# TUMFTM/RadarGNN

Hardware: AMD Instinct MI355X
Metric: radar frames/sec (graph-build + GNN fwd) (higher is better)
Workload: dtype f32 (dense layers: fp32 operands split into 2 f16 terms after an exact power-of-two pre-scale, 3 f16 MFMA products per fp32 product, fp32 accumulate -- more accurate than fp32 MFMA against float64, tests/test_gpu_f16x2.py; RGNN_NO_F16X2=1 selects 3 bf16 terms / 6 products, RGNN_LINEAR_FP32=1 v_mfma_; 1 GPU; C2: per GPU 64 RadarScenes-shaped frames x 3000 pts, radius graph r=1.0, node feats [rcs,velocity_vector,time_index,degree], edge feats [relative_position], 4-layer MPNNConv [224,224,128,64] + emb MLPs + both heads, train-mode BatchNorm, max aggr; frames_per_gpu=64, points_per_gpu=192000, edges_per_gpu=799078, ranks_in_process_group=1

## Files before the change

### radargnn_amd/csrc/mpnn_tiles.hip

```cpp
#include "common.h"
#include <stdlib.h>
#include <type_traits>

namespace {

constexpr int MT_THREADS = 256;
constexpr int MT_WAVES = MT_THREADS / 64;
constexpr int MT_QUEUE_INTS = 8 * 16;

typedef float mt_f32x16 __attribute__((ext_vector_type(16)));
typedef __bf16 mt_bf16x8 __attribute__((ext_vector_type(8)));
typedef unsigned int mt_u32x4 __attribute__((ext_vector_type(4)));

__global__ __launch_bounds__(256) void k_tiles_zero_empty(const int32_t* __restrict__ rowptr, const int32_t* __restrict__ order,
                                                         int64_t n, int d, float* __restrict__ out, int64_t ldo) {
  const int lane = threadIdx.x & 63;
  const int64_t p = (int64_t)blockIdx.x * MT_WAVES + (threadIdx.x >> 6);
  if (p >= n || rowptr[p + 1] != rowptr[p]) return;
  const int64_t node = order ? order[p] : p;
  for (int c = lane; c < d; c += 64) out[node * ldo + c] = 0.f;
}

__device__ __forceinline__ void mt_split3(float x, unsigned& t1, unsigned& t2, unsigned& t3) {
  t1 = __float_as_uint(x) & 0xffff0000u;
  const float r = x - __uint_as_float(t1);
  t2 = __float_as_uint(r) & 0xffff0000u;
  const float r2 = r - __uint_as_float(t2);
  t3 = __float_as_uint(r2) & 0xffff0000u;
}
__device__ __forceinline__ unsigned mt_pack(unsigned lo, unsigned hi) { return (lo >> 16) | hi; }
__device__ __forceinline__ void mt_split_row(const float (&x)[8], mt_u32x4& p1, mt_u32x4& p2, mt_u32x4& p3) {
  unsigned t1[8], t2[8], t3[8];
#pragma unroll
  for (int k = 0; k < 8; k++) mt_split3(x[k], t1[k], t2[k], t3[k]);
  p1 = mt_u32x4{mt_pack(t1[0], t1[1]), mt_pack(t1[2], t1[3]), mt_pack(t1[4], t1[5]), mt_pack(t1[6], t1[7])};
  p2 = mt_u32x4{mt_pack(t2[0], t2[1]), mt_pack(t2[2], t2[3]), mt_pack(t2[4], t2[5]), mt_pack(t2[6], t2[7])};
  p3 = mt_u32x4{mt_pack(t3[0], t3[1]), mt_pack(t3[2], t3[3]), mt_pack(t3[4], t3[5]), mt_pack(t3[6], t3[7])};
}

}

namespace {

constexpr int WN_SLOTS = 512;
constexpr int WN_THREADS = 256;
typedef int wn_i32x4 __attribute__((ext_vector_type(4)));

struct WinParams {
  const float* p_bias;
  const float* Q; int ldq4; int q_bytes;
  const mt_u32x4* wplanes;
  const float* ea; int de; int ea_vec;
  int n_win;
  const int32_t* n_win_dev;
  const int32_t* plan; int plan_bytes;
  int off_misc;
  int off_eid;
  int off_lrow;
  int off_urow;
  int off_tgt;
  int32_t* queue;
  int d; int n_ct;
  float* out; int ldo4; int o_bytes;
  float* out_absmax;
  int abl;
};

__device__ __forceinline__ void wn_dma16(wn_i32x4 rsrc, int voff, int soff, unsigned lds_base) {
  asm volatile(
      "s_mov_b32 m0, %3\n\t"
      "s_nop 0\n\t"
      "buffer_load_dwordx4 %0, %1, %2 offen lds"
      :
      : "v"(voff), "s"(rsrc), "s"(soff), "s"(lds_base)
      : "memory");
}

__global__ __launch_bounds__(256) void k_win_wplanes(const float* __restrict__ We, int ldwe, int de, int d, int n_ct, const float* __restrict__ p_bias,
                                                     mt_u32x4* __restrict__ planes) {
  const int c = blockIdx.x * blockDim.x + threadIdx.x;
  if (c >= n_ct * 32) return;
  float w[8];
#pragma unroll
  for (int k = 0; k < 8; k++) w[k] = (c < d && k < de) ? We[(int64_t)c * ldwe + k] : 0.f;
  mt_u32x4 p1, p2, p3;
  mt_split_row(w, p1, p2, p3);
  mt_u32x4* t = planes + (c >> 5) * 128 + (c & 31);
  t[0] = p1; t[32] = p2; t[64] = p3;
  t[96] = mt_u32x4{__float_as_uint((p_bias != nullptr && c < d) ? p_bias[c] : 0.f), 0u, 0u, 0u};
}

constexpr int WN_PAD = 4;
constexpr int WN_GPT = 16 / WN_PAD;
constexpr int WN_GPS = 64 / WN_PAD;
constexpr int WN_TMAX = 512 / WN_PAD;
static_assert(WN_PAD == 2 || WN_PAD == 4, "segments are padded to 2 or 4 slots");
constexpr int WN_NOEND = (int)0x80000000u;
constexpr int WN_UMAX = 176;
constexpr int WN_ROWBUF = WN_UMAX * 128;

__device__ __forceinline__ void wn_wait_leaving(int n) {
  switch (n) {
#define WN_W(N) case N: asm volatile("s_waitcnt vmcnt(" #N ")" ::: "memory"); break;
    WN_W(1) WN_W(2) WN_W(3) WN_W(4) WN_W(5) WN_W(6) WN_W(7) WN_W(8) WN_W(9) WN_W(10) WN_W(11) WN_W(12) WN_W(13) WN_W(14) WN_W(15) WN_W(16)
    WN_W(17) WN_W(18) WN_W(19) WN_W(20) WN_W(21) WN_W(22) WN_W(23) WN_W(24) WN_W(25) WN_W(26) WN_W(27) WN_W(28) WN_W(29) WN_W(30) WN_W(31) WN_W(32)
#undef WN_W
    default: asm volatile("s_waitcnt vmcnt(0)" ::: "memory"); break;
  }
}

constexpr bool WN_WARM = false;
constexpr int WN_BBUF = 32 * 64;

constexpr int WN_DESC = 2 * WN_UMAX * 4 + 2048 + 512 + 8 * WN_GPS * 4 + 64;
static_assert((2 * WN_UMAX * 128 + 2 * 32 * 64 + WN_DESC + 16 + 511) / 512 * 512 * 3 <= 160 * 1024, "k_mpnn_win: LDS of three work-groups per CU");
constexpr int WN_LDS = 2 * WN_ROWBUF + 2 * WN_BBUF + WN_DESC + 16;

template <bool AMAX>
__global__ __launch_bounds__(WN_THREADS) __attribute__((amdgpu_waves_per_eu(3, 3))) void k_mpnn_win(const WinParams p) {
  extern __shared__ __attribute__((aligned(16))) char smem[];
  char* bstage = smem + 2 * WN_ROWBUF;
  int* urowtab = (int*)(bstage + 2 * WN_BBUF);
  int* eidtab = urowtab + 2 * WN_UMAX;
  const uint8_t* lrowtab = (const uint8_t*)(eidtab + 512);
  int* tgttab = eidtab + 512 + 128;
  int* misctab = tgttab + 8 * WN_GPS;
  int* bcast = misctab + 16;
  const unsigned rows_lds = (unsigned)(uintptr_t)(__attribute__((address_space(3))) char*)smem;
  const unsigned b_lds = rows_lds + 2 * WN_ROWBUF;
  const unsigned desc_lds = b_lds + 2 * WN_BBUF;
  const int tid = threadIdx.x, lane = tid & 63, wave = __builtin_amdgcn_readfirstlane(tid >> 6), half = lane >> 5, col = lane & 31, col4 = col * 4;
  const int xcd = blockIdx.x & 7;
  const int n_win = min(p.n_win, __builtin_amdgcn_readfirstlane(p.n_win_dev[0]));
  const int i_lo = (int)((int64_t)n_win * xcd / 8), i_hi = (int)((int64_t)n_win * (xcd + 1) / 8);
  int32_t* ticket = p.queue + xcd * 16;
  wn_i32x4 rq, rw, rp;
  {
    const uint64_t a = (uint64_t)p.Q;
    rq.x = __builtin_amdgcn_readfirstlane((int)(uint32_t)a);
    rq.y = __builtin_amdgcn_readfirstlane((int)(uint32_t)((a >> 32) & 0xffff));
    rq.z = __builtin_amdgcn_readfirstlane(p.q_bytes);
    rq.w = 0x00020000;
    const uint64_t b = (uint64_t)p.wplanes;
    rw.x = __builtin_amdgcn_readfirstlane((int)(uint32_t)b);
    rw.y = __builtin_amdgcn_readfirstlane((int)(uint32_t)((b >> 32) & 0xffff));
    rw.z = __builtin_amdgcn_readfirstlane(p.n_ct * WN_BBUF);
    rw.w = 0x00020000;
    const uint64_t c = (uint64_t)p.plan;
    rp.x = __builtin_amdgcn_readfirstlane((int)(uint32_t)c);
    rp.y = __builtin_amdgcn_readfirstlane((int)(uint32_t)((c >> 32) & 0xffff));
    rp.z = __builtin_amdgcn_readfirstlane(p.plan_bytes);
    rp.w = 0x00020000;
  }
  const int rA = lane & 31, hA = (rA >> 2) & 1, iA = ((rA >> 3) << 2) | (rA & 3);
  const int my_stream = 2 * wave + half;
  float amax = 0.f;

  auto desc_dma = [&](const int w, const int up) {
    if (wave == 0) {
      if (lane < WN_UMAX / 4) wn_dma16(rp, lane * 16, __builtin_amdgcn_readfirstlane(p.off_urow + w * (WN_UMAX * 4)),
                                       (unsigned)__builtin_amdgcn_readfirstlane((int)(desc_lds + up * (WN_UMAX * 4))));
    } else if (wave == 1) {
      wn_dma16(rp, lane * 16, __builtin_amdgcn_readfirstlane(p.off_eid + w * 2048), desc_lds + 8 * WN_UMAX);
      wn_dma16(rp, lane * 16, __builtin_amdgcn_readfirstlane(p.off_eid + w * 2048 + 1024), desc_lds + 8 * WN_UMAX + 1024);
    } else if (wave == 2) {
      if (lane < 32) wn_dma16(rp, lane * 16, __builtin_amdgcn_readfirstlane(p.off_lrow + w * 512), desc_lds + 8 * WN_UMAX + 2048);
    } else {
      if (lane < 2 * WN_GPS) wn_dma16(rp, lane * 16, __builtin_amdgcn_readfirstlane(p.off_tgt + w * (32 * WN_GPS)), desc_lds + 8 * WN_UMAX + 2560);
      if (lane < 4) wn_dma16(rp, lane * 16, __builtin_amdgcn_readfirstlane(p.off_misc + w * 64), desc_lds + 8 * WN_UMAX + 2560 + 32 * WN_GPS);
    }
  };
  auto stage = [&](const int ct, const int st, const int up, const int nU8) {
    const unsigned base = rows_lds + st * WN_ROWBUF;
    const int* ut = urowtab + up * WN_UMAX;
    for (int k = wave; k < nU8; k += 4)
      wn_dma16(rq, (int)__umul24((unsigned)ut[8 * k + (lane >> 3)], (unsigned)p.ldq4) + (lane & 7) * 16, __builtin_amdgcn_readfirstlane(ct * 128),
               (unsigned)__builtin_amdgcn_readfirstlane((int)(base + k * 1024)));
    if (wave == 1) {
      const unsigned bb = b_lds + st * WN_BBUF;
      wn_dma16(rw, lane * 16, __builtin_amdgcn_readfirstlane(ct * WN_BBUF), (unsigned)__builtin_amdgcn_readfirstlane((int)bb));
      wn_dma16(rw, lane * 16 + 1024, __builtin_amdgcn_readfirstlane(ct * WN_BBUF), (unsigned)__builtin_amdgcn_readfirstlane((int)(bb + 1024)));
    }
  };

  if (tid == 0) { bcast[0] = i_lo + atomicAdd(ticket, 1); bcast[1] = i_lo + atomicAdd(ticket, 1); }
  __syncthreads();
  int win = bcast[0];
  int up = 0;
  int gp = 0;
  bool staged = false;
  if (win < i_hi) desc_dma(win, 0);
  asm volatile("s_waitcnt vmcnt(0)" ::: "memory");
  __syncthreads();
  for (;;) {
    if (win >= i_hi) {
      if (tid == 0) {
        const int wgs = (int)(gridDim.x >> 3);
        if (atomicAdd(ticket + 1, 1) == wgs - 1) { ticket[0] = 0; ticket[1] = 0; }
      }
      break;
    }
    const int nxt = bcast[1];
    const int nU = misctab[0];
    const int nU8 = (nU + 7) >> 3;
    int nt = 0;
    unsigned anyend = 0;
    mt_u32x4 a1[4], a2[4], a3[4];
    int aoff[4][16];
    int tv = WN_NOEND;
    if (nU != 0) {
      const uint8_t* m8 = (const uint8_t*)(misctab + 1);
      nt = max((int)m8[2 * wave], (int)m8[2 * wave + 1]);
      const uint8_t* e4 = m8 + 8 + my_stream * 4;
      const unsigned endbits = (unsigned)e4[0] | ((unsigned)e4[1] << WN_GPT) | ((unsigned)e4[2] << (2 * WN_GPT)) | ((unsigned)e4[3] << (3 * WN_GPT));
      anyend = (unsigned)__builtin_amdgcn_readlane((int)endbits, 0) | (unsigned)__builtin_amdgcn_readlane((int)endbits, 32);
      const int gj = lane & (WN_GPS - 1);
      tv = ((endbits >> gj) & 1u) ? tgttab[my_stream * WN_GPS + gj] * p.ldo4 : WN_NOEND;
#pragma unroll
      for (int t = 0; t < 4; t++) {
        const int e = eidtab[(2 * wave + hA) * 64 + t * 16 + iA];
        float z[8];
        if (p.ea_vec) {
          const float4 mine = *(const float4*)(p.ea + (int64_t)e * 8 + half * 4);
          const float4 other = make_float4(__shfl_xor(mine.x, 32, 64), __shfl_xor(mine.y, 32, 64), __shfl_xor(mine.z, 32, 64), __shfl_xor(mine.w, 32, 64));
          const float4 lo = half ? other : mine, hi = half ? mine : other;
          z[0] = lo.x; z[1] = lo.y; z[2] = lo.z; z[3] = lo.w; z[4] = hi.x; z[5] = hi.y; z[6] = hi.z; z[7] = hi.w;
        } else {
#pragma unroll
          for (int k = 0; k < 8; k++) z[k] = (k < p.de) ? p.ea[(int64_t)e * p.de + k] : 0.f;
        }
        mt_u32x4 t3;
        mt_split_row(z, a1[t], a2[t], t3);
        a3[t] = half ? a1[t] : t3;
      }
      const mt_u32x4* lt = (const mt_u32x4*)(lrowtab + my_stream * 64);
#pragma unroll
      for (int t = 0; t < 4; t++) {
        const mt_u32x4 w4 = lt[t];
#pragma unroll
        for (int i = 0; i < 16; i++) {
          const unsigned w = w4[i >> 2];
          const unsigned r = (i & 3) == 3 ? (w >> 24) : ((w >> (8 * (i & 3))) & 0xffu);
          aoff[t][i] = (int)(rows_lds + (r << 7)) + col4;
          asm volatile("" : "+v"(aoff[t][i]));
        }
      }
    }
    __syncthreads();
    if (tid == 0) bcast[1] = i_lo + atomicAdd(ticket, 1);
    if (nU == 0) {
      if (nxt < i_hi) desc_dma(nxt, up ^ 1);
      asm volatile("s_waitcnt vmcnt(0)" ::: "memory");
      __syncthreads();
      win = nxt; up ^= 1; staged = false;
      continue;
    }
    const int nst = __builtin_popcount(anyend & ((nt >= 4) ? (WN_GPT == 8 ? 0xffffffffu : 0xffffu) : ((1u << (WN_GPT * nt)) - 1u)));
    if (!staged) stage(0, gp, up, nU8);
    bool staged_next = false;

    auto tile_pass = [&](const int ct, auto stage_c) {
      constexpr int ST = decltype(stage_c)::value;
      if (ct == 0 || (p.abl & 1)) asm volatile("s_waitcnt vmcnt(0)" ::: "memory");
      else wn_wait_leaving(nst);
      __syncthreads();
      if (ct == 0 && nxt < i_hi) desc_dma(nxt, up ^ 1);
      if (ct + 1 < p.n_ct) {
        if (!(p.abl & 1)) stage(ct + 1, ST ^ 1, up, nU8);
      } else if (ct > 0 && nxt < i_hi && !(p.abl & 1)) {
        const int nUn = misctab[0];
        if (nUn != 0) { stage(0, ST ^ 1, up ^ 1, (nUn + 7) >> 3); staged_next = true; }
      }
      const mt_u32x4* bl = (const mt_u32x4*)(bstage + ST * WN_BBUF);
      const mt_u32x4 bxc = bl[(half ? 32 : 0) + col], byc = bl[(half ? 64 : 0) + col];
      const float biasc = __uint_as_float(bl[96 + col].x);
      const int voffc = (ct * 32 + col < p.d && !(p.abl & 4)) ? col4 : 0x7ffffff0;
      const __amdgpu_buffer_rsrc_t ro_l = __builtin_amdgcn_make_buffer_rsrc((void*)((char*)p.out + ct * 128), (short)0, p.o_bytes - ct * 128, 0x00020000);
      float rn = -INFINITY;
      asm volatile("" : "+v"(tv), "+s"(anyend));
#pragma unroll
      for (int t = 0; t < 4; t++) {
        if (t < nt && !(p.abl & 2)) {
          mt_f32x16 c;
#pragma unroll
          for (int i = 0; i < 16; i++) c[i] = *(const __attribute__((address_space(3))) float*)(uintptr_t)(unsigned)(aoff[t][i] + ST * WN_ROWBUF);
          c = __builtin_amdgcn_mfma_f32_32x32x16_bf16(__builtin_bit_cast(mt_bf16x8, a3[t]), __builtin_bit_cast(mt_bf16x8, byc), c, 0, 0, 0);
          c = __builtin_amdgcn_mfma_f32_32x32x16_bf16(__builtin_bit_cast(mt_bf16x8, a2[t]), __builtin_bit_cast(mt_bf16x8, bxc), c, 0, 0, 0);
          c = __builtin_amdgcn_mfma_f32_32x32x16_bf16(__builtin_bit_cast(mt_bf16x8, a1[t]), __builtin_bit_cast(mt_bf16x8, bxc), c, 0, 0, 0);
#pragma unroll
          for (int g = 0; g < WN_GPT; g++) {
            rn = __builtin_fmaxf(__builtin_fmaxf(rn, c[WN_PAD * g]), c[WN_PAD * g + 1]);
            if (WN_PAD == 4) rn = __builtin_fmaxf(__builtin_fmaxf(rn, c[WN_PAD * g + 2]), c[WN_PAD * g + 3]);
            if ((anyend >> (WN_GPT * t + g)) & 1u) {
              const float v = rn + biasc;
              const int toA = __builtin_amdgcn_readlane(tv, WN_GPT * t + g), toB = __builtin_amdgcn_readlane(tv, 32 + WN_GPT * t + g);
              const int tog = half ? toB : toA;
              asm volatile("buffer_store_dword %0, %1, %2, 0 offen nt" : : "v"(v), "v"((unsigned)tog + (unsigned)voffc), "s"(ro_l) : "memory");
              if (AMAX) amax = fmaxf(amax, fabsf(v));
              rn = (tog >= 0) ? -INFINITY : rn;
            }
          }
        }
      }
    };
    float amax_full = 0.f;
    for (int ct = 0; ct < p.n_ct; ct++) {
      const bool partial = AMAX && (ct + 1) * 32 > p.d;
      if (partial) { amax_full = amax; amax = 0.f; }
      if ((gp + ct) & 1) tile_pass(ct, std::integral_constant<int, 1>());
      else tile_pass(ct, std::integral_constant<int, 0>());
      if (partial) amax = fmaxf(amax_full, (ct * 32 + col < p.d) ? amax : 0.f);
    }
    if (p.n_ct < 2) {
      asm volatile("s_waitcnt vmcnt(0)" ::: "memory");
      __syncthreads();
    }
    gp = (gp + p.n_ct) & 1;
    win = nxt; up ^= 1; staged = staged_next;
  }
  if (AMAX) {
#pragma unroll
    for (int o = 32; o > 0; o >>= 1) amax = fmaxf(amax, __shfl_xor(amax, o, 64));
    if (lane == 0)
      atomicMax((unsigned int*)p.out_absmax + ((blockIdx.x * 4 + wave) & (RGNN_BOUND_SLOTS - 1)), __float_as_uint(amax));
  }
}

constexpr int WN_BIG = 64;

constexpr int WN_SEG = 512;
struct WinPlanLayout {
  int n_win, n_seg;
  int64_t off_assign, off_segcnt, off_segbase, off_wend, off_pdeg, off_wstart, off_left, off_leftcnt, off_queue, off_misc, off_tgt, off_eid, off_lrow, off_urow,
      off_wplanes, total_ints;
};
WinPlanLayout win_layout(int64_t n, int64_t n_edges) {
  WinPlanLayout L;
  L.n_seg = (int)((n + WN_SEG - 1) / WN_SEG);
  L.n_win = (int)((n_edges + 3 * n) / 256 + L.n_seg + 2);
  int64_t o = 16;
  auto take = [&](int64_t ints) { const int64_t at = o; o = (o + ints + 15) / 16 * 16; return at; };
  L.off_assign = take(n + 1); L.off_segcnt = take(L.n_seg + 1); L.off_segbase = take(L.n_seg + 2);
  L.off_wend = take(L.n_win + 1);
  L.off_pdeg = take(n + 1); L.off_wstart = take(L.n_win + 1); L.off_left = take(n + 1); L.off_leftcnt = take(4);
  L.off_queue = take(MT_QUEUE_INTS); L.off_misc = take(16 * (int64_t)L.n_win);
  L.off_tgt = take(8 * WN_GPS * (int64_t)L.n_win); L.off_eid = take(512 * (int64_t)L.n_win); L.off_lrow = take(128 * (int64_t)L.n_win);
  L.off_urow = take(WN_UMAX * (int64_t)L.n_win); L.off_wplanes = take(16 * 64 * 32);
  L.total_ints = o;
  return L;
}

__global__ __launch_bounds__(256) void k_win_pdeg(const int32_t* __restrict__ rowptr, int64_t n, int32_t* __restrict__ pdeg,
                                                 int32_t* __restrict__ left, int32_t* __restrict__ leftcnt, int32_t* __restrict__ queue) {
  const int64_t p = (int64_t)blockIdx.x * blockDim.x + threadIdx.x;
  if (p < MT_QUEUE_INTS) queue[p] = 0;
  if (p > n) return;
  if (p == n) { pdeg[p] = 0; return; }
  const int d = rowptr[p + 1] - rowptr[p];
  const int pd = (d + WN_PAD - 1) & ~(WN_PAD - 1);
  if (pd > WN_BIG) left[atomicAdd(leftcnt, 1)] = (int32_t)p;
  pdeg[p] = (pd > WN_BIG) ? 0 : pd;
}
__global__ __launch_bounds__(64) void k_win_greedy(const int32_t* __restrict__ pdeg, int64_t n, int32_t* __restrict__ assign,
                                                  int32_t* __restrict__ segcnt) {
  __shared__ int spd[WN_SEG];
  __shared__ int sas[WN_SEG];
  const int seg = blockIdx.x, lane = threadIdx.x;
  const int64_t p0 = (int64_t)seg * WN_SEG;
  const int cnt = (int)min((int64_t)WN_SEG, n - p0);
  for (int i = lane; i < cnt; i += 64) spd[i] = pdeg[p0 + i];
  __syncthreads();
  {
    int fill = 0;
    int win = 0, any = 0;
    for (int ib = 0; ib < cnt; ib += 64) {
      const int mine_pd = (ib + lane < cnt) ? spd[ib + lane] : 0;
      int mine_as = -1;
      const int nb = min(64, cnt - ib);
      for (int j = 0; j < nb; j++) {
        const int pd = __builtin_amdgcn_readlane(mine_pd, j);
        if (pd == 0) continue;
        const unsigned long long fits = __ballot(lane < 8 && fill + pd <= 64);
        int b = 0;
        if (fits == 0) { win++; fill = 0; }
        else b = __builtin_ctzll(fits);
        const int off = __builtin_amdgcn_readlane(fill, b);
        if (lane == b) fill += pd;
        any = 1;
        if (lane == j) mine_as = (win << 16) | (b * 64 + off);
      }
      if (ib + lane < cnt) sas[ib + lane] = mine_as;
    }
    if (lane == 0) segcnt[seg] = any ? win + 1 : 0;
  }
  __syncthreads();
  for (int i = lane; i < cnt; i += 64) assign[p0 + i] = sas[i];
}
__global__ __launch_bounds__(1024) void k_win_segbase(const int32_t* __restrict__ segcnt, int n_seg, int32_t* __restrict__ segbase) {
  __shared__ int part[1024];
  const int t = threadIdx.x;
  const int per = (n_seg + 1023) / 1024;
  int sum = 0;
  for (int i = t * per; i < min(n_seg, (t + 1) * per); i++) sum += segcnt[i];
  part[t] = sum;
  __syncthreads();
  for (int o = 1; o < 1024; o <<= 1) {
    const int v = t >= o ? part[t - o] : 0;
    __syncthreads();
    part[t] += v;
    __syncthreads();
  }
  int run = part[t] - sum;
  for (int i = t * per; i < min(n_seg, (t + 1) * per); i++) { segbase[i] = run; run += segcnt[i]; }
  if (t == 1023) segbase[n_seg] = part[1023];
}
__global__ __launch_bounds__(256) void k_win_starts(const int32_t* __restrict__ assign, const int32_t* __restrict__ segbase, int64_t n, int n_seg,
                                                   int n_win, int32_t* __restrict__ wstart, int32_t* __restrict__ wend) {
  const int64_t p = (int64_t)blockIdx.x * blockDim.x + threadIdx.x;
  if (p >= n) return;
  const int a = assign[p];
  if (a < 0) return;
  const int seg = (int)(p / WN_SEG);
  const int w = segbase[seg] + (a >> 16);
  if (w >= n_win) return;
  if ((a & 0xffff) == 0) wstart[w] = (int32_t)p;
  atomicMax(&wend[w], (int32_t)p + 1);
}

__global__ __launch_bounds__(256) void k_win_pack(const int32_t* __restrict__ rowptr, const int32_t* __restrict__ src,
                                                 const int32_t* __restrict__ order, const int32_t* __restrict__ pdeg,
                                                 const int32_t* __restrict__ assign, const int32_t* __restrict__ segbase,
                                                 const int32_t* __restrict__ wstart, const int32_t* __restrict__ wend, int n_win,
                                                 int32_t* __restrict__ misc_out, int32_t* __restrict__ tgt_out,
                                                 int32_t* __restrict__ eid_out, uint8_t* __restrict__ lrow_out, int32_t* __restrict__ urow_out,
                                                 int32_t* __restrict__ left, int32_t* __restrict__ leftcnt) {
  __shared__ int s_src[4][512];
  __shared__ int s_key[4][1024];
  __shared__ int s_val[4][1024];
  __shared__ short s_assign[4][WN_TMAX];
  __shared__ int s_pos[4][WN_TMAX];
  __shared__ int s_pd[4][WN_TMAX];
  __shared__ int s_e0[4][WN_TMAX];
  __shared__ int s_misc[4][16];
  __shared__ int s_end[4][32];
  const int lane = threadIdx.x & 63, wv = threadIdx.x >> 6;
  const int w = blockIdx.x * 4 + wv;
  if (w >= n_win) return;
  const int p1 = wend[w], p0 = p1 > 0 ? wstart[w] : 0;
  int* ssrc = s_src[wv]; int* skey = s_key[wv]; int* sval = s_val[wv]; short* sas = s_assign[wv]; int* spos = s_pos[wv]; int* spd = s_pd[wv]; int* se0 = s_e0[wv]; int* misc = s_misc[wv]; int* send = s_end[wv];
  const int64_t wb = (int64_t)w * 512;
  if (p1 == 0) {
    if (lane < 16) misc_out[(int64_t)w * 16 + lane] = 0;
    return;
  }
  for (int i = lane; i < 512; i += 64) { ssrc[i] = -1; eid_out[wb + i] = 0; lrow_out[wb + i] = 0; }
  for (int i = lane; i < 1024; i += 64) skey[i] = -1;
  for (int i = lane; i < 8 * WN_GPS; i += 64) tgt_out[(int64_t)w * (8 * WN_GPS) + i] = 0;
  if (lane < 32) send[lane] = 0;
  if (lane == 0) misc[9] = 0;
  __builtin_amdgcn_s_waitcnt(0);
  __builtin_amdgcn_wave_barrier();
  for (int pb = p0; pb < p1; pb += 64) {
    const int p = pb + lane;
    const int a = p < p1 ? assign[p] : -1;
    const bool mine = a >= 0 && segbase[p / WN_SEG] + (a >> 16) == w;
    const unsigned long long m = __ballot(mine);
    const int base = misc[9];
    const int j = base + __popcll(m & ((1ull << lane) - 1ull));
    if (mine) {
      if (j < WN_TMAX) { spos[j] = p; spd[j] = pdeg[p]; se0[j] = rowptr[p]; sas[j] = (short)(a & 0xffff); }
      else left[atomicAdd(leftcnt, 1)] = p;
    }
    __builtin_amdgcn_s_waitcnt(0);
    __builtin_amdgcn_wave_barrier();
    if (lane == 0) misc[9] = min(base + __popcll(m), WN_TMAX);
    __builtin_amdgcn_s_waitcnt(0);
    __builtin_amdgcn_wave_barrier();
  }
  const int cnt = misc[9];
  if (lane < 8) misc[lane] = 0;
  __builtin_amdgcn_s_waitcnt(0);
  __builtin_amdgcn_wave_barrier();
  for (int i = lane; i < cnt; i += 64) atomicMax(&misc[sas[i] >> 6], (sas[i] & 63) + spd[i]);
  for (int i = lane; i < cnt; i += 64) {
    const int at = sas[i], p = spos[i], e0 = se0[i], pd = spd[i];
    const int d = rowptr[p + 1] - e0;
    for (int q = 0; q < pd; q++) {
      const int e = e0 + min(q, d - 1);
      eid_out[wb + at + q] = e;
      ssrc[at + q] = src[e];
    }
    const int gi = ((at & 63) + pd - WN_PAD) / WN_PAD, b = at >> 6;
    atomicOr(&send[b * 4 + gi / WN_GPT], 1 << (gi % WN_GPT));
    tgt_out[(int64_t)w * (8 * WN_GPS) + b * WN_GPS + gi] = order ? order[p] : p;
  }
  __builtin_amdgcn_s_waitcnt(0);
  __builtin_amdgcn_wave_barrier();
  if (lane == 0) misc[8] = 0;
  for (int i = lane; i < 512; i += 64) {
    const int s_ = ssrc[i];
    if (s_ < 0) continue;
    unsigned h = ((unsigned)s_ * 2654435761u) >> 22;
    for (;;) {
      const int prev = atomicCAS(&skey[h], -1, s_);
      if (prev == -1 || prev == s_) break;
      h = (h + 1) & 1023;
    }
  }
  __builtin_amdgcn_s_waitcnt(0);
  __builtin_amdgcn_wave_barrier();
  for (int i = lane; i < 1024; i += 64)
    if (skey[i] >= 0) sval[i] = atomicAdd(&misc[8], 1);
  __builtin_amdgcn_s_waitcnt(0);
  __builtin_amdgcn_wave_barrier();
  const int nU = misc[8];
  if (nU > WN_UMAX) {
    for (int i = lane; i < cnt; i += 64) left[atomicAdd(leftcnt, 1)] = spos[i];
    if (lane < 16) misc_out[(int64_t)w * 16 + lane] = 0;
    return;
  }
  for (int i = lane; i < 1024; i += 64)
    if (skey[i] >= 0) urow_out[(int64_t)w * WN_UMAX + sval[i]] = skey[i];
  for (int i = lane; i < 512; i += 64) {
    const int s_ = ssrc[i];
    if (s_ < 0) continue;
    unsigned h = ((unsigned)s_ * 2654435761u) >> 22;
    while (skey[h] != s_) h = (h + 1) & 1023;
    lrow_out[wb + i] = (uint8_t)sval[h];
  }
  if (lane < 8 && nU + lane < ((nU + 7) & ~7)) urow_out[(int64_t)w * WN_UMAX + nU + lane] = 0;
  uint8_t* m8 = (uint8_t*)(misc_out + (int64_t)w * 16);
  if (lane == 0) misc_out[(int64_t)w * 16] = nU;
  if (lane < 8) m8[4 + lane] = (uint8_t)((misc[lane] + 15) >> 4);
  if (lane < 32) m8[12 + lane] = (uint8_t)send[lane];
  if (lane < 5) m8[44 + 4 * lane] = 0, m8[45 + 4 * lane] = 0, m8[46 + 4 * lane] = 0, m8[47 + 4 * lane] = 0;
}

__global__ __launch_bounds__(256) void k_win_leftover(const float* __restrict__ p_bias, const float* __restrict__ Q, int64_t ldq,
                                                     const float* __restrict__ We, int ldwe, const float* __restrict__ ea, int de,
                                                     const int32_t* __restrict__ rowptr, const int32_t* __restrict__ src,
                                                     const int32_t* __restrict__ order, const int32_t* __restrict__ left,
                                                     const int32_t* __restrict__ leftcnt, int d, float* __restrict__ out, int64_t ldo,
                                                     float* __restrict__ out_absmax) {
  const int lane = threadIdx.x & 63, wv = threadIdx.x >> 6;
  const int n_left = *leftcnt;
  if (n_left == 0) return;
  float amax = 0.f;
  for (int c0 = 0; c0 < d; c0 += 512) {
    const int cw = c0 + 128 * wv;
    if (cw >= d) continue;
    float w[2][8];
    bool ok[2];
#pragma unroll
    for (int j = 0; j < 2; j++) {
      const int c = cw + 64 * j + lane;
      ok[j] = c < d;
#pragma unroll
      for (int k = 0; k < 8; k++) w[j][k] = (ok[j] && k < de) ? We[(int64_t)c * ldwe + k] : 0.f;
    }
    for (int64_t i = blockIdx.x; i < n_left; i += gridDim.x) {
      const int p = left[i];
      const int e0 = rowptr[p], e1 = rowptr[p + 1];
      const int64_t node = order ? order[p] : p;
      float m[2] = {-INFINITY, -INFINITY};
      for (int eb = e0; eb < e1; eb += 64) {
        const int el = min(eb + lane, e1 - 1);
        const int my_src = src[el];
        float my_z[8];
#pragma unroll
        for (int k = 0; k < 8; k++) my_z[k] = k < de ? ea[(int64_t)el * de + k] : 0.f;
        const int nb = min(64, e1 - eb);
        for (int q = 0; q < nb; q += 8) {
          float v[8][2];
          int jj[8];
#pragma unroll
          for (int u = 0; u < 8; u++) {
            jj[u] = min(q + u, nb - 1);
            const int64_t r = (int64_t)__builtin_amdgcn_readlane(my_src, jj[u]) * ldq + cw + lane;
#pragma unroll
            for (int j = 0; j < 2; j++) v[u][j] = ok[j] ? Q[r + 64 * j] : 0.f;
          }
#pragma unroll
          for (int u = 0; u < 8; u++) {
            float z[8];
#pragma unroll
            for (int k = 0; k < 8; k++) z[k] = __builtin_bit_cast(float, __builtin_amdgcn_readlane(__builtin_bit_cast(int, my_z[k]), jj[u]));
#pragma unroll
            for (int j = 0; j < 2; j++) {
#pragma unroll
              for (int k = 0; k < 8; k++) v[u][j] = __builtin_fmaf(w[j][k], z[k], v[u][j]);
              m[j] = fmaxf(m[j], v[u][j]);
            }
          }
        }
      }
#pragma unroll
      for (int j = 0; j < 2; j++) {
        if (!ok[j]) continue;
        const int c = cw + 64 * j + lane;
        const float o = m[j] + (p_bias ? p_bias[c] : 0.f);
        out[node * ldo + c] = o;
        amax = fmaxf(amax, fabsf(o));
      }
    }
  }
  if (out_absmax != nullptr) {
#pragma unroll
    for (int o = 32; o > 0; o >>= 1) amax = fmaxf(amax, __shfl_xor(amax, o, 64));
    if (lane == 0 && amax > 0.f)
      atomicMax((unsigned int*)out_absmax + ((blockIdx.x * 4 + wv) & (RGNN_BOUND_SLOTS - 1)), __float_as_uint(amax));
  }
}

}

extern "C" int64_t rgnn_mpnn_win_plan_ints(int64_t n, int64_t n_edges) { return win_layout(n, n_edges).total_ints; }
extern "C" void rgnn_mpnn_win_plan_counters(int64_t n, int64_t n_edges, int64_t* leftover_word, int64_t* windows_word) {
  const WinPlanLayout L = win_layout(n, n_edges);
  *leftover_word = L.off_leftcnt;
  *windows_word = L.off_segbase + L.n_seg;
}

extern "C" int rgnn_mpnn_win_plan(const int32_t* rowptr_t, const int32_t* src_sorted, const int32_t* node_order, int64_t n, int64_t n_edges,
                                  int32_t* plan, rgnn_stream_t stream) {
  RGNN_CHECK_ARG(rowptr_t && plan && n >= 0 && n_edges >= 0, "bad arguments");
  RGNN_CHECK_ARG(n_edges == 0 || src_sorted, "null src_sorted");
  RGNN_CHECK_ARG((((uintptr_t)plan) & 15) == 0, "plan must be 16-byte aligned");
  if (n == 0) return RGNN_OK;
  const WinPlanLayout L = win_layout(n, n_edges);
  hipStream_t s = (hipStream_t)stream;
  hipMemsetAsync(plan + L.off_leftcnt, 0, 16, s);
  hipLaunchKernelGGL(k_win_pdeg, dim3(rgnn_blocks(n + 1 > MT_QUEUE_INTS ? n + 1 : MT_QUEUE_INTS, 256)), dim3(256), 0, s, rowptr_t, n, plan + L.off_pdeg,
                     plan + L.off_left, plan + L.off_leftcnt, plan + L.off_queue);
  hipMemsetAsync(plan + L.off_wend, 0, 4 * (size_t)(L.n_win + 1), s);
  hipLaunchKernelGGL(k_win_greedy, dim3(L.n_seg), dim3(64), 0, s, (const int32_t*)(plan + L.off_pdeg), n, plan + L.off_assign, plan + L.off_segcnt);
  hipLaunchKernelGGL(k_win_segbase, dim3(1), dim3(1024), 0, s, (const int32_t*)(plan + L.off_segcnt), L.n_seg, plan + L.off_segbase);
  hipLaunchKernelGGL(k_win_starts, dim3(rgnn_blocks(n, 256)), dim3(256), 0, s, (const int32_t*)(plan + L.off_assign),
                     (const int32_t*)(plan + L.off_segbase), n, L.n_seg, L.n_win, plan + L.off_wstart, plan + L.off_wend);
  hipLaunchKernelGGL(k_win_pack, dim3(rgnn_blocks(L.n_win, 4)), dim3(256), 0, s, rowptr_t, src_sorted, node_order,
                     (const int32_t*)(plan + L.off_pdeg), (const int32_t*)(plan + L.off_assign), (const int32_t*)(plan + L.off_segbase),
                     (const int32_t*)(plan + L.off_wstart), (const int32_t*)(plan + L.off_wend), L.n_win, plan + L.off_misc,
                     plan + L.off_tgt, plan + L.off_eid, (uint8_t*)(plan + L.off_lrow),
                     plan + L.off_urow, plan + L.off_left, plan + L.off_leftcnt);
  RGNN_CHECK_LAUNCH();
  return RGNN_OK;
}

extern "C" int64_t rgnn_mpnn_win_wplanes_bytes(int32_t d) { return d < 1 ? -1 : (int64_t)((d + 31) / 32) * WN_BBUF; }

extern "C" int rgnn_mpnn_win_wplanes(const float* We, int64_t ldwe, int32_t de, int32_t d, const float* p_bias, void* planes,
                                     rgnn_stream_t stream) {
  RGNN_CHECK_ARG(planes && d >= 1 && de >= 0 && de <= 8 && (de == 0 || We) && (((uintptr_t)planes) & 15) == 0, "bad arguments");
  const int n_ct = (d + 31) / 32;
  hipLaunchKernelGGL(k_win_wplanes, dim3(rgnn_blocks(n_ct * 32, 256)), dim3(256), 0, (hipStream_t)stream, We, (int)ldwe, de, d, n_ct, p_bias,
                     (mt_u32x4*)planes);
  RGNN_CHECK_LAUNCH();
  return RGNN_OK;
}

extern "C" int rgnn_mpnn_aggregate_win(const float* p_bias, const float* Q, int64_t ldq, const float* We, int64_t ldwe,
                                       const float* edge_attr_sorted, int32_t de, const int32_t* rowptr_t, const int32_t* src_sorted,
                                       const int32_t* node_order, int32_t* plan, int64_t n, int64_t n_edges, int32_t d, float* out,
                                       int64_t ldo, int32_t flags, float* out_absmax, const void* wplanes, rgnn_stream_t stream) {
  if (n == 0) return RGNN_OK;
  RGNN_CHECK_ARG(Q && rowptr_t && plan && out && d >= 1, "bad arguments");
  RGNN_CHECK_ARG((flags & ~RGNN_MPNN_SKIP_EMPTY_ROWS) == 0, "unknown flags");
  RGNN_CHECK_ARG(de == 0 || ((We || wplanes) && edge_attr_sorted), "edge attributes given without weights");
  RGNN_CHECK_ARG((((uintptr_t)wplanes) & 15) == 0, "operand image not 16-byte aligned");
  const int64_t q_bytes = ((n - 1) * ldq + d) * 4, o_bytes = ((n - 1) * ldo + d) * 4;
  if (de > 8 || d > 2048 || n >= ((int64_t)1 << 24) || ldq * 4 >= ((int64_t)1 << 24) || q_bytes >= ((int64_t)1 << 31) ||
      o_bytes >= ((int64_t)1 << 31) || (ldq % 4) != 0 || (((uintptr_t)Q) & 15) != 0 || win_layout(n, n_edges).total_ints * 4 >= ((int64_t)1 << 31)) {
    rgnn_set_error("rgnn_mpnn_aggregate_win: shape not covered (de %d, d %d, n %lld, ldq %lld)", de, d, (long long)n, (long long)ldq);
    return RGNN_ERR_UNSUPPORTED;
  }
  hipStream_t s = (hipStream_t)stream;
  if (!(flags & RGNN_MPNN_SKIP_EMPTY_ROWS))
    hipLaunchKernelGGL(k_tiles_zero_empty, dim3(rgnn_blocks(n, MT_WAVES)), dim3(256), 0, s, rowptr_t, node_order, n, d, out, ldo);
  if (n_edges > 0) {
    const WinPlanLayout L = win_layout(n, n_edges);
    WinParams p;
    p.p_bias = p_bias; p.Q = Q; p.ldq4 = (int)(ldq * 4); p.q_bytes = (int)q_bytes;
    p.wplanes = wplanes ? (const mt_u32x4*)wplanes : (const mt_u32x4*)(plan + L.off_wplanes); p.ea = edge_attr_sorted; p.de = de;
    p.ea_vec = (de == 8 && (((uintptr_t)edge_attr_sorted) & 15) == 0) ? 1 : 0;
    p.n_win = L.n_win; p.n_win_dev = plan + L.off_segbase + L.n_seg;
    p.plan = plan; p.plan_bytes = (int)(L.total_ints * 4);
    p.off_misc = (int)(L.off_misc * 4); p.off_eid = (int)(L.off_eid * 4); p.off_lrow = (int)(L.off_lrow * 4); p.off_urow = (int)(L.off_urow * 4); p.off_tgt = (int)(L.off_tgt * 4);
    p.queue = plan + L.off_queue;
    p.d = d; p.n_ct = (d + 31) / 32; p.out = out; p.ldo4 = (int)(ldo * 4); p.o_bytes = (int)o_bytes; p.out_absmax = out_absmax;
    p.abl = RGNN_ENV("RGNN_MPNN_WIN_ABL") ? atoi(RGNN_ENV("RGNN_MPNN_WIN_ABL")) : 0;
    if (!wplanes)
      hipLaunchKernelGGL(k_win_wplanes, dim3(rgnn_blocks(p.n_ct * 32, 256)), dim3(256), 0, s, We, (int)ldwe, de, d, p.n_ct, p_bias,
                         (mt_u32x4*)(plan + L.off_wplanes));
    const size_t lds = WN_LDS;
    static RgnnOncePerDevice attr_once;
    if (attr_once.first()) {
      hipFuncSetAttribute((const void*)k_mpnn_win<true>, hipFuncAttributeMaxDynamicSharedMemorySize, (int)lds);
      hipFuncSetAttribute((const void*)k_mpnn_win<false>, hipFuncAttributeMaxDynamicSharedMemorySize, (int)lds);
    }
    static const int per_cu = RGNN_ENV("RGNN_MPNN_WIN_WG_PER_CU") ? atoi(RGNN_ENV("RGNN_MPNN_WIN_WG_PER_CU")) : 3;
    int64_t blocks = L.n_win;
    if (blocks > 256 * per_cu) blocks = 256 * per_cu;
    blocks = (blocks + 7) / 8 * 8;
    rgnn_prof_begin(s);
    if (out_absmax) hipLaunchKernelGGL((k_mpnn_win<true>), dim3((unsigned)blocks), dim3(WN_THREADS), lds, s, p);
    else hipLaunchKernelGGL((k_mpnn_win<false>), dim3((unsigned)blocks), dim3(WN_THREADS), lds, s, p);
    rgnn_prof_end(s);
    hipLaunchKernelGGL(k_win_leftover, dim3(2048), dim3(256), 0, s, p_bias, Q, ldq, We, (int)ldwe, edge_attr_sorted, de, rowptr_t, src_sorted,
                       node_order, (const int32_t*)(plan + L.off_left), (const int32_t*)(plan + L.off_leftcnt), d, out, ldo, out_absmax);
  }
  RGNN_CHECK_LAUNCH();
  return RGNN_OK;
}
```

Measured before the change: 32000 frames/s.

## Fuse window-plan build into fewer kernels with SWAR greedy packing

Drops the separate pdeg, starts kernels and two memsets by having the greedy kernel read rowptr directly, compact big nodes per segment, and emit a per-segment table of window start/end. The segbase scan then writes window bounds, the leftover list and the queue reset. The greedy bin-fit becomes a packed-byte add/carry test over 8 bins instead of a ballot per node. This removes launches and per-node atomics from graph-build planning, at the cost of more serial work in the single-block scan kernel and more complex packing logic.

Result: faster. 32650 frames/s (median of 6 runs) (+2.0%).

```diff
diff --git a/radargnn_amd/csrc/mpnn_tiles.hip b/radargnn_amd/csrc/mpnn_tiles.hip
--- a/radargnn_amd/csrc/mpnn_tiles.hip
+++ b/radargnn_amd/csrc/mpnn_tiles.hip
@@ -329,10 +329,13 @@
 constexpr int WN_BIG = 64;
 
 constexpr int WN_SEG = 512;
+constexpr int WN_SEGWIN = 64;
+static_assert((WN_SEG - 1) / 8 + 1 <= WN_SEGWIN, "a segment's table of windows is too short");
+static_assert(WN_SEG % 64 == 0 && WN_SEG < (1 << 16), "a segment is whole waves of positions; a table word packs two positions of it");
 struct WinPlanLayout {
   int n_win, n_seg;
-  int64_t off_assign, off_segcnt, off_segbase, off_wend, off_pdeg, off_wstart, off_left, off_leftcnt, off_queue, off_misc, off_tgt, off_eid, off_lrow, off_urow,
-      off_wplanes, total_ints;
+  int64_t off_assign, off_segcnt, off_segbase, off_wend, off_big, off_wstart, off_left, off_leftcnt, off_queue, off_misc, off_tgt, off_eid, off_lrow, off_urow,
+      off_wplanes, off_bigcnt, off_wtab, total_ints;
 };
 WinPlanLayout win_layout(int64_t n, int64_t n_edges) {
   WinPlanLayout L;
@@ -342,94 +345,130 @@
   auto take = [&](int64_t ints) { const int64_t at = o; o = (o + ints + 15) / 16 * 16; return at; };
   L.off_assign = take(n + 1); L.off_segcnt = take(L.n_seg + 1); L.off_segbase = take(L.n_seg + 2);
   L.off_wend = take(L.n_win + 1);
-  L.off_pdeg = take(n + 1); L.off_wstart = take(L.n_win + 1); L.off_left = take(n + 1); L.off_leftcnt = take(4);
+  L.off_big = take(n + 1); L.off_wstart = take(L.n_win + 1); L.off_left = take(n + 1); L.off_leftcnt = take(4);
   L.off_queue = take(MT_QUEUE_INTS); L.off_misc = take(16 * (int64_t)L.n_win);
   L.off_tgt = take(8 * WN_GPS * (int64_t)L.n_win); L.off_eid = take(512 * (int64_t)L.n_win); L.off_lrow = take(128 * (int64_t)L.n_win);
   L.off_urow = take(WN_UMAX * (int64_t)L.n_win); L.off_wplanes = take(16 * 64 * 32);
+  L.off_bigcnt = take(L.n_seg + 1); L.off_wtab = take(WN_SEGWIN * (int64_t)L.n_seg);
   L.total_ints = o;
   return L;
 }
 
-__global__ __launch_bounds__(256) void k_win_pdeg(const int32_t* __restrict__ rowptr, int64_t n, int32_t* __restrict__ pdeg,
-                                                 int32_t* __restrict__ left, int32_t* __restrict__ leftcnt, int32_t* __restrict__ queue) {
-  const int64_t p = (int64_t)blockIdx.x * blockDim.x + threadIdx.x;
-  if (p < MT_QUEUE_INTS) queue[p] = 0;
-  if (p > n) return;
-  if (p == n) { pdeg[p] = 0; return; }
-  const int d = rowptr[p + 1] - rowptr[p];
-  const int pd = (d + WN_PAD - 1) & ~(WN_PAD - 1);
-  if (pd > WN_BIG) left[atomicAdd(leftcnt, 1)] = (int32_t)p;
-  pdeg[p] = (pd > WN_BIG) ? 0 : pd;
-}
-__global__ __launch_bounds__(64) void k_win_greedy(const int32_t* __restrict__ pdeg, int64_t n, int32_t* __restrict__ assign,
-                                                  int32_t* __restrict__ segcnt) {
-  __shared__ int spd[WN_SEG];
-  __shared__ int sas[WN_SEG];
+__global__ __launch_bounds__(64) void k_win_greedy(const int32_t* __restrict__ rowptr, int64_t n, int32_t* __restrict__ assign,
+                                                  int32_t* __restrict__ segcnt, int32_t* __restrict__ wtab, int32_t* __restrict__ big,
+                                                  int32_t* __restrict__ bigcnt) {
+  __shared__ unsigned srep[WN_SEG];
+  __shared__ int sfirst[WN_SEGWIN];
+  __shared__ int slast[WN_SEGWIN];
+  static_assert(WN_SEGWIN == 64, "one lane per table word");
   const int seg = blockIdx.x, lane = threadIdx.x;
   const int64_t p0 = (int64_t)seg * WN_SEG;
   const int cnt = (int)min((int64_t)WN_SEG, n - p0);
-  for (int i = lane; i < cnt; i += 64) spd[i] = pdeg[p0 + i];
+  sfirst[lane] = 0; slast[lane] = 0;
+  int lo[WN_SEG / 64], hi[WN_SEG / 64];
+#pragma unroll
+  for (int c = 0; c < WN_SEG / 64; c++) {
+    const int i = c * 64 + lane;
+    lo[c] = i < cnt ? rowptr[p0 + i] : 0;
+    hi[c] = i < cnt ? rowptr[p0 + i + 1] : 0;
+  }
+  int nbig = 0;
+#pragma unroll
+  for (int c = 0; c < WN_SEG / 64; c++) {
+    const int i = c * 64 + lane;
+    const int pd = (hi[c] - lo[c] + WN_PAD - 1) & ~(WN_PAD - 1);
+    const bool isbig = pd > WN_BIG;
+    const unsigned long long m = __ballot(isbig);
+    if (isbig) big[p0 + nbig + __popcll(m & ((1ull << lane) - 1ull))] = (int32_t)(p0 + i);
+    nbig += __popcll(m);
+    srep[i] = (pd > 0 && !isbig) ? (unsigned)pd * 0x01010101u + 0x3F3F3F3Fu : 0u;
+  }
   __syncthreads();
-  {
-    int fill = 0;
-    int win = 0, any = 0;
-    for (int ib = 0; ib < cnt; ib += 64) {
-      const int mine_pd = (ib + lane < cnt) ? spd[ib + lane] : 0;
-      int mine_as = -1;
-      const int nb = min(64, cnt - ib);
-      for (int j = 0; j < nb; j++) {
-        const int pd = __builtin_amdgcn_readlane(mine_pd, j);
-        if (pd == 0) continue;
-        const unsigned long long fits = __ballot(lane < 8 && fill + pd <= 64);
-        int b = 0;
-        if (fits == 0) { win++; fill = 0; }
-        else b = __builtin_ctzll(fits);
-        const int off = __builtin_amdgcn_readlane(fill, b);
-        if (lane == b) fill += pd;
-        any = 1;
-        if (lane == j) mine_as = (win << 16) | (b * 64 + off);
-      }
-      if (ib + lane < cnt) sas[ib + lane] = mine_as;
-    }
-    if (lane == 0) segcnt[seg] = any ? win + 1 : 0;
+  unsigned long long fill = 0;
+  int win16 = 0;
+  for (int ib = 0; ib < cnt; ib += 64) {
+    const unsigned mine_rep = srep[ib + lane];
+    const unsigned mine_pd = (mine_rep & 0xff) - 0x3F;
+    int mine_as = -1;
+#pragma unroll
+    for (int j = 0; j < 64; j++) {
+      const unsigned r = __builtin_amdgcn_readlane(mine_rep, j);
+      if (r == 0) continue;
+      const unsigned pd = __builtin_amdgcn_readlane(mine_pd, j);
+      const unsigned tlo = (unsigned)fill + r, thi = (unsigned)(fill >> 32) + r;
+      unsigned long long fit = ~(((unsigned long long)thi << 32) | tlo) & 0x8080808080808080ull;
+      if (__builtin_expect(fit == 0, 0)) { win16 += 1 << 16; fill = 0; fit = 0x80; }
+      const int sh = __builtin_ctzll(fit) & 56;
+      const int as = win16 | ((sh << 3) + (int)((fill >> sh) & 0xff));
+      fill += (unsigned long long)pd << sh;
+      if (__builtin_amdgcn_inverse_ballot_w64(1ull << j)) mine_as = as;
+    }
+    const bool placed = mine_as >= 0;
+    const unsigned long long above = lane < 63 ? __ballot(placed) >> (lane + 1) : 0ull;
+    const int next_as = __shfl(mine_as, above ? lane + 1 + __builtin_ctzll(above) : lane, 64);
+    if (placed) {
+      const int k = mine_as >> 16;
+      if ((mine_as & 0xffff) == 0) sfirst[k] = ib + lane;
+      if (above == 0 || (next_as >> 16) != k) slast[k] = ib + lane + 1;
+    }
+    if (ib + lane < cnt) assign[p0 + ib + lane] = mine_as;
   }
   __syncthreads();
-  for (int i = lane; i < cnt; i += 64) assign[p0 + i] = sas[i];
-}
-__global__ __launch_bounds__(1024) void k_win_segbase(const int32_t* __restrict__ segcnt, int n_seg, int32_t* __restrict__ segbase) {
+  const int made = fill ? (win16 >> 16) + 1 : 0;
+  wtab[(int64_t)seg * WN_SEGWIN + lane] = lane < made ? (sfirst[lane] | (slast[lane] << 16)) : 0;
+  if (lane == 0) { segcnt[seg] = made; bigcnt[seg] = nbig; }
+}
+__global__ __launch_bounds__(1024) void k_win_segbase(const int32_t* __restrict__ segcnt, const int32_t* __restrict__ bigcnt,
+                                                     const int32_t* __restrict__ wtab, const int32_t* __restrict__ big, int n_seg, int n_win,
+                                                     int32_t* __restrict__ segbase, int32_t* __restrict__ wstart, int32_t* __restrict__ wend,
+                                                     int32_t* __restrict__ left, int32_t* __restrict__ leftcnt, int32_t* __restrict__ queue) {
   __shared__ int part[1024];
+  __shared__ int bpart[1024];
   const int t = threadIdx.x;
+  if (t < MT_QUEUE_INTS) queue[t] = 0;
   const int per = (n_seg + 1023) / 1024;
-  int sum = 0;
-  for (int i = t * per; i < min(n_seg, (t + 1) * per); i++) sum += segcnt[i];
-  part[t] = sum;
+  int sum = 0, bsum = 0;
+  for (int i = t * per; i < min(n_seg, (t + 1) * per); i++) { sum += segcnt[i]; bsum += bigcnt[i]; }
+  part[t] = sum; bpart[t] = bsum;
   __syncthreads();
   for (int o = 1; o < 1024; o <<= 1) {
-    const int v = t >= o ? part[t - o] : 0;
+    const int v = t >= o ? part[t - o] : 0, bv = t >= o ? bpart[t - o] : 0;
     __syncthreads();
-    part[t] += v;
+    part[t] += v; bpart[t] += bv;
     __syncthreads();
   }
-  int run = part[t] - sum;
-  for (int i = t * per; i < min(n_seg, (t + 1) * per); i++) { segbase[i] = run; run += segcnt[i]; }
+  int run = part[t] - sum, brun = bpart[t] - bsum;
+  for (int i = t * per; i < min(n_seg, (t + 1) * per); i++) {
+    const int c = segcnt[i], bc = bigcnt[i];
+    const int p0 = i * WN_SEG;
+    segbase[i] = run;
+    for (int k0 = 0; k0 < c; k0 += 8) {
+      int word[8];
+#pragma unroll
+      for (int k = 0; k < 8; k++) word[k] = k0 + k < c ? wtab[(int64_t)i * WN_SEGWIN + k0 + k] : 0;
+#pragma unroll
+      for (int k = 0; k < 8; k++) {
+        const int w = run + k0 + k;
+        if (k0 + k < c && w < n_win) { wstart[w] = p0 + (word[k] & 0xffff); wend[w] = p0 + (int)((unsigned)word[k] >> 16); }
+      }
+    }
+    for (int k0 = 0; k0 < bc; k0 += 8) {
+      int pos[8];
+#pragma unroll
+      for (int k = 0; k < 8; k++) pos[k] = k0 + k < bc ? big[(int64_t)p0 + k0 + k] : 0;
+#pragma unroll
+      for (int k = 0; k < 8; k++)
+        if (k0 + k < bc) left[brun + k0 + k] = pos[k];
+    }
+    run += c; brun += bc;
+  }
   if (t == 1023) segbase[n_seg] = part[1023];
-}
-__global__ __launch_bounds__(256) void k_win_starts(const int32_t* __restrict__ assign, const int32_t* __restrict__ segbase, int64_t n, int n_seg,
-                                                   int n_win, int32_t* __restrict__ wstart, int32_t* __restrict__ wend) {
-  const int64_t p = (int64_t)blockIdx.x * blockDim.x + threadIdx.x;
-  if (p >= n) return;
-  const int a = assign[p];
-  if (a < 0) return;
-  const int seg = (int)(p / WN_SEG);
-  const int w = segbase[seg] + (a >> 16);
-  if (w >= n_win) return;
-  if ((a & 0xffff) == 0) wstart[w] = (int32_t)p;
-  atomicMax(&wend[w], (int32_t)p + 1);
+  if (t < 4) leftcnt[t] = t == 0 ? bpart[1023] : 0;
 }
 
 __global__ __launch_bounds__(256) void k_win_pack(const int32_t* __restrict__ rowptr, const int32_t* __restrict__ src,
-                                                 const int32_t* __restrict__ order, const int32_t* __restrict__ pdeg,
-                                                 const int32_t* __restrict__ assign, const int32_t* __restrict__ segbase,
+                                                 const int32_t* __restrict__ order, const int32_t* __restrict__ assign,
+                                                 const int32_t* __restrict__ segbase, int n_seg,
                                                  const int32_t* __restrict__ wstart, const int32_t* __restrict__ wend, int n_win,
                                                  int32_t* __restrict__ misc_out, int32_t* __restrict__ tgt_out,
                                                  int32_t* __restrict__ eid_out, uint8_t* __restrict__ lrow_out, int32_t* __restrict__ urow_out,
@@ -446,13 +485,13 @@
   const int lane = threadIdx.x & 63, wv = threadIdx.x >> 6;
   const int w = blockIdx.x * 4 + wv;
   if (w >= n_win) return;
-  const int p1 = wend[w], p0 = p1 > 0 ? wstart[w] : 0;
   int* ssrc = s_src[wv]; int* skey = s_key[wv]; int* sval = s_val[wv]; short* sas = s_assign[wv]; int* spos = s_pos[wv]; int* spd = s_pd[wv]; int* se0 = s_e0[wv]; int* misc = s_misc[wv]; int* send = s_end[wv];
   const int64_t wb = (int64_t)w * 512;
-  if (p1 == 0) {
+  if (w >= segbase[n_seg]) {
     if (lane < 16) misc_out[(int64_t)w * 16 + lane] = 0;
     return;
   }
+  const int p0 = wstart[w], p1 = wend[w];
   for (int i = lane; i < 512; i += 64) { ssrc[i] = -1; eid_out[wb + i] = 0; lrow_out[wb + i] = 0; }
   for (int i = lane; i < 1024; i += 64) skey[i] = -1;
   for (int i = lane; i < 8 * WN_GPS; i += 64) tgt_out[(int64_t)w * (8 * WN_GPS) + i] = 0;
@@ -468,7 +507,8 @@
     const int base = misc[9];
     const int j = base + __popcll(m & ((1ull << lane) - 1ull));
     if (mine) {
-      if (j < WN_TMAX) { spos[j] = p; spd[j] = pdeg[p]; se0[j] = rowptr[p]; sas[j] = (short)(a & 0xffff); }
+      const int e0 = rowptr[p];
+      if (j < WN_TMAX) { spos[j] = p; spd[j] = (rowptr[p + 1] - e0 + WN_PAD - 1) & ~(WN_PAD - 1); se0[j] = e0; sas[j] = (short)(a & 0xffff); }
       else left[atomicAdd(leftcnt, 1)] = p;
     }
     __builtin_amdgcn_s_waitcnt(0);
@@ -629,16 +669,13 @@
   if (n == 0) return RGNN_OK;
   const WinPlanLayout L = win_layout(n, n_edges);
   hipStream_t s = (hipStream_t)stream;
-  hipMemsetAsync(plan + L.off_leftcnt, 0, 16, s);
-  hipLaunchKernelGGL(k_win_pdeg, dim3(rgnn_blocks(n + 1 > MT_QUEUE_INTS ? n + 1 : MT_QUEUE_INTS, 256)), dim3(256), 0, s, rowptr_t, n, plan + L.off_pdeg,
-                     plan + L.off_left, plan + L.off_leftcnt, plan + L.off_queue);
-  hipMemsetAsync(plan + L.off_wend, 0, 4 * (size_t)(L.n_win + 1), s);
-  hipLaunchKernelGGL(k_win_greedy, dim3(L.n_seg), dim3(64), 0, s, (const int32_t*)(plan + L.off_pdeg), n, plan + L.off_assign, plan + L.off_segcnt);
-  hipLaunchKernelGGL(k_win_segbase, dim3(1), dim3(1024), 0, s, (const int32_t*)(plan + L.off_segcnt), L.n_seg, plan + L.off_segbase);
-  hipLaunchKernelGGL(k_win_starts, dim3(rgnn_blocks(n, 256)), dim3(256), 0, s, (const int32_t*)(plan + L.off_assign),
-                     (const int32_t*)(plan + L.off_segbase), n, L.n_seg, L.n_win, plan + L.off_wstart, plan + L.off_wend);
+  hipLaunchKernelGGL(k_win_greedy, dim3(L.n_seg), dim3(64), 0, s, rowptr_t, n, plan + L.off_assign, plan + L.off_segcnt, plan + L.off_wtab,
+                     plan + L.off_big, plan + L.off_bigcnt);
+  hipLaunchKernelGGL(k_win_segbase, dim3(1), dim3(1024), 0, s, (const int32_t*)(plan + L.off_segcnt), (const int32_t*)(plan + L.off_bigcnt),
+                     (const int32_t*)(plan + L.off_wtab), (const int32_t*)(plan + L.off_big), L.n_seg, L.n_win, plan + L.off_segbase,
+                     plan + L.off_wstart, plan + L.off_wend, plan + L.off_left, plan + L.off_leftcnt, plan + L.off_queue);
   hipLaunchKernelGGL(k_win_pack, dim3(rgnn_blocks(L.n_win, 4)), dim3(256), 0, s, rowptr_t, src_sorted, node_order,
-                     (const int32_t*)(plan + L.off_pdeg), (const int32_t*)(plan + L.off_assign), (const int32_t*)(plan + L.off_segbase),
+                     (const int32_t*)(plan + L.off_assign), (const int32_t*)(plan + L.off_segbase), L.n_seg,
                      (const int32_t*)(plan + L.off_wstart), (const int32_t*)(plan + L.off_wend), L.n_win, plan + L.off_misc,
                      plan + L.off_tgt, plan + L.off_eid, (uint8_t*)(plan + L.off_lrow),
                      plan + L.off_urow, plan + L.off_left, plan + L.off_leftcnt);
```
